# laurabragagnolo/SkelSplat

Hardware: AMD Instinct MI355X
Metric: rendered+backpropagated views/s (differentiable skeletal-Gaussian rasterizer fwd+bwd) (higher is better)
Workload: dtype f32

## Files before the change

### skelsplat_amd/csrc/sks_geom_bwd.inc

```
struct GeomBwdArgs {
    int P, C, W, H;
    unsigned flags;
    const float* vms;
    const float* pms;
    const float* means;
    const float* opac;
    const float* scales;
    const float* rots;
    const float* cov3Dp;
    float smod;
    const int* radii;
    const float* accum;
    int nsplit;
    const double* gt_totals;
    double* loss_sums;
    float* packed;
    float* dmeans3D;
    float* dmeans2D;
    float* dopacity;
    float* dscales;
    float* drots;
    float* dcov3D;
    float* dfeat;
    const uint4* rect = nullptr;
// ... 79 lines not shown
__device__ __forceinline__ void geom_bwd_issue16(const GeomBwdArgs& a, int v, int idx, GeomBwdRaw& r)
{
    const size_t o = (size_t)v * a.P + (idx < a.P ? idx : 0);
    const float* acc = a.accum + o * BWD_SPLITS * (NACC + a.C);
#pragma unroll
    for (int j = 0; j < NACC + 1; j++)
#pragma unroll
        for (int i = 0; i < 4; i++) r.q[j][i] = reinterpret_cast<const float4*>(acc + j * BWD_SPLITS)[i];
}
__device__ __forceinline__ void geom_bwd_sum16(const GeomBwdArgs& a, int idx, const GeomBwdRaw& r, float (&g)[NACC], double& pS,
                                               double& pN)
{
#pragma unroll
    for (int j = 0; j < NACC - 1; j++) {
        float t = 0.0f;
#pragma unroll
        for (int i = 0; i < 4; i++) t += (r.q[j][i].x + r.q[j][i].y) + (r.q[j][i].z + r.q[j][i].w);
        g[j] = t;
    }
    g[NACC - 1] = 0.0f;
    pS = 0.0;
    pN = 0.0;
    if (a.loss_sums && idx < a.P) {
#pragma unroll
        for (int i = 0; i < 4; i++) {
            pS += (double)r.q[7][i].x; pS += (double)r.q[7][i].y; pS += (double)r.q[7][i].z; pS += (double)r.q[7][i].w;
            pN += (double)r.q[8][i].x; pN += (double)r.q[8][i].y; pN += (double)r.q[8][i].z; pN += (double)r.q[8][i].w;
        }
    }
}

struct GeomBwdIn {
    int radius;
    float mean[3], p[7], opac;
};
__device__ __forceinline__ void geom_bwd_fetch(const GeomBwdArgs& a, int v, int idx, GeomBwdIn& in)
{
    const size_t o = (size_t)v * a.P + idx;
    in.radius = a.radii[o];
    in.mean[0] = a.means[3 * idx]; in.mean[1] = a.means[3 * idx + 1]; in.mean[2] = a.means[3 * idx + 2];
    if (a.cov3Dp) {
#pragma unroll
        for (int i = 0; i < 6; i++) in.p[i] = a.cov3Dp[6 * idx + i];
        in.p[6] = 0.0f;
    } else {
        in.p[0] = a.scales[3 * idx]; in.p[1] = a.scales[3 * idx + 1]; in.p[2] = a.scales[3 * idx + 2];
        in.p[3] = a.rots[4 * idx]; in.p[4] = a.rots[4 * idx + 1]; in.p[5] = a.rots[4 * idx + 2]; in.p[6] = a.rots[4 * idx + 3];
    }
    in.opac = a.opac[idx];
}

template <bool PRE = false, class VT = ViewTan>
__device__ __forceinline__ void geom_bwd_finish(const GeomBwdArgs& a, const VT& vt, int v, int idx, const float (&g)[NACC],
                                                double n_view, const GeomBwdIn* pre = nullptr)
{
    const size_t o = (size_t)v * a.P + idx;
    float dmean[3] = { 0, 0, 0 }, dcov[6] = { 0, 0, 0, 0, 0, 0 }, dscale[3] = { 0, 0, 0 }, dq[4] = { 0, 0, 0, 0 };
    float sc[3] = { 0, 0, 0 }, q[4] = { 1, 0, 0, 0 }, qnorm = 1.0f;
    float dop = g[5];
    const float dm2x = g[0], dm2y = g[1];

    if ((PRE ? pre->radius : a.radii[o]) > 0) {
        const float* V = a.vms + 16 * v;
        const float* proj = a.pms + 16 * v;
        const float tan_fovx = vt.x[v], tan_fovy = vt.y[v];
        const float h_y = vt.h[v] / (2.0f * tan_fovy);
        const float h_x = vt.w[v] / (2.0f * tan_fovx);
        const float mean[3] = { PRE ? pre->mean[0] : a.means[3 * idx], PRE ? pre->mean[1] : a.means[3 * idx + 1], PRE ? pre->mean[2] : a.means[3 * idx + 2] };
        float cov3D[6];
        if (a.cov3Dp) {
#pragma unroll
            for (int i = 0; i < 6; i++) cov3D[i] = PRE ? pre->p[i] : a.cov3Dp[6 * idx + i];
        } else {
            const float rs[3] = { PRE ? pre->p[0] : a.scales[3 * idx], PRE ? pre->p[1] : a.scales[3 * idx + 1], PRE ? pre->p[2] : a.scales[3 * idx + 2] };
            const float rq[4] = { PRE ? pre->p[3] : a.rots[4 * idx], PRE ? pre->p[4] : a.rots[4 * idx + 1], PRE ? pre->p[5] : a.rots[4 * idx + 2],
                                  PRE ? pre->p[6] : a.rots[4 * idx + 3] };
            const Activated ac = activate(a.flags & SKS_RAW_PARAMS, 0.0f, rs, rq);
            sc[0] = ac.s[0]; sc[1] = ac.s[1]; sc[2] = ac.s[2];
            q[0] = ac.q[0]; q[1] = ac.q[1]; q[2] = ac.q[2]; q[3] = ac.q[3];
            qnorm = ac.qnorm;
            computeCov3D(sc, a.smod, q, cov3D);
        }
        const float dL_dconic[3] = { g[2], g[3], g[4] };
        Cov2D c;
        cov2d(mean, h_x, h_y, tan_fovx, tan_fovy, cov3D, V, c);
        const float* t = c.t;
        const float x_grad_mul = (c.txtz < -c.limx || c.txtz > c.limx) ? 0 : 1;
        const float y_grad_mul = (c.tytz < -c.limy || c.tytz > c.limy) ? 0 : 1;
        const M3& T = c.T;
        const M3& Wm = c.W;
        const M3& Vrk = c.Vrk;
        float c_xx = c.cov.m[0][0], c_xy = c.cov.m[0][1], c_yy = c.cov.m[1][1];
        constexpr float h_var = 0.3f;
        float d_inside_root = 0.f;
        const bool aa = a.flags & SKS_ANTIALIASING;
        if (aa) {
            const float det_cov = c_xx * c_yy - c_xy * c_xy;
            c_xx += h_var;
            c_yy += h_var;
            const float det_cov_plus_h_cov = c_xx * c_yy - c_xy * c_xy;
            const float h_convolution_scaling = sqrtf(fmaxf(0.000025f, det_cov / det_cov_plus_h_cov));
            const float dL_dopacity_v = dop;
            const float op_raw = PRE ? pre->opac : a.opac[idx];
            const float d_h_convolution_scaling = dL_dopacity_v * ((a.flags & SKS_RAW_PARAMS) ? 1.0f / (1.0f + expf_fixed(-op_raw)) : op_raw);
            dop = dL_dopacity_v * h_convolution_scaling;
            d_inside_root = (det_cov / det_cov_plus_h_cov) <= 0.000025f ? 0.f : d_h_convolution_scaling / (2 * h_convolution_scaling);
        } else {
// ... 38 lines not shown
        const float dL_dJ11 = Wm.m[1][0] * dL_dT10 + Wm.m[1][1] * dL_dT11 + Wm.m[1][2] * dL_dT12;
        const float dL_dJ12 = Wm.m[2][0] * dL_dT10 + Wm.m[2][1] * dL_dT11 + Wm.m[2][2] * dL_dT12;
        const float tz = 1.f / t[2];
        const float tz2 = tz * tz;
        const float tz3 = tz2 * tz;
        const float dL_dtx = x_grad_mul * -h_x * tz2 * dL_dJ02;
        const float dL_dty = y_grad_mul * -h_y * tz2 * dL_dJ12;
        float dL_dtz = -h_x * tz2 * dL_dJ00 - h_y * tz2 * dL_dJ11 + (2 * h_x * t[0]) * tz3 * dL_dJ02 + (2 * h_y * t[1]) * tz3 * dL_dJ12;
        dL_dtz -= g[6] / (t[2] * t[2]);
        dmean[0] = V[0] * dL_dtx + V[1] * dL_dty + V[2] * dL_dtz;
        dmean[1] = V[4] * dL_dtx + V[5] * dL_dty + V[6] * dL_dtz;
        dmean[2] = V[8] * dL_dtx + V[9] * dL_dty + V[10] * dL_dtz;
        float m_hom[4];
        transformPoint4x4(mean, proj, m_hom);
        const float m_w = 1.0f / (m_hom[3] + 0.0000001f);
        const float mul1 = (proj[0] * mean[0] + proj[4] * mean[1] + proj[8] * mean[2] + proj[12]) * m_w * m_w;
        const float mul2 = (proj[1] * mean[0] + proj[5] * mean[1] + proj[9] * mean[2] + proj[13]) * m_w * m_w;
        dmean[0] += (proj[0] * m_w - proj[3] * mul1) * dm2x + (proj[1] * m_w - proj[3] * mul2) * dm2y;
        dmean[1] += (proj[4] * m_w - proj[7] * mul1) * dm2x + (proj[5] * m_w - proj[7] * mul2) * dm2y;
        dmean[2] += (proj[8] * m_w - proj[11] * mul1) * dm2x + (proj[9] * m_w - proj[11] * mul2) * dm2y;
        if (!a.cov3Dp) {
            const float r = q[0], x = q[1], y = q[2], z = q[3];
            const M3 R = quatR(q);
            M3 S = {};
            const float s[3] = { a.smod * sc[0], a.smod * sc[1], a.smod * sc[2] };
            S.m[0][0] = s[0]; S.m[1][1] = s[1]; S.m[2][2] = s[2];
            const M3 M = m3mul(S, R);
            M3 dS;
            dS.m[0][0] = dcov[0]; dS.m[0][1] = 0.5f * dcov[1]; dS.m[0][2] = 0.5f * dcov[2];
            dS.m[1][0] = 0.5f * dcov[1]; dS.m[1][1] = dcov[3]; dS.m[1][2] = 0.5f * dcov[4];
            dS.m[2][0] = 0.5f * dcov[2]; dS.m[2][1] = 0.5f * dcov[4]; dS.m[2][2] = dcov[5];
            M3 M2;
#pragma unroll
            for (int cc = 0; cc < 3; cc++)
#pragma unroll
                for (int rr = 0; rr < 3; rr++) M2.m[cc][rr] = 2.0f * M.m[cc][rr];
            const M3 dL_dM = m3mul(M2, dS);
            const M3 Rt = m3T(R);
            M3 dMt = m3T(dL_dM);
#pragma unroll
            for (int k = 0; k < 3; k++)
                dscale[k] = Rt.m[k][0] * dMt.m[k][0] + Rt.m[k][1] * dMt.m[k][1] + Rt.m[k][2] * dMt.m[k][2];
#pragma unroll
            for (int k = 0; k < 3; k++)
#pragma unroll
                for (int rr = 0; rr < 3; rr++) dMt.m[k][rr] *= s[k];
            dq[0] = 2 * z * (dMt.m[0][1] - dMt.m[1][0]) + 2 * y * (dMt.m[2][0] - dMt.m[0][2]) + 2 * x * (dMt.m[1][2] - dMt.m[2][1]);
            dq[1] = 2 * y * (dMt.m[1][0] + dMt.m[0][1]) + 2 * z * (dMt.m[2][0] + dMt.m[0][2]) + 2 * r * (dMt.m[1][2] - dMt.m[2][1]) - 4 * x * (dMt.m[2][2] + dMt.m[1][1]);
            dq[2] = 2 * x * (dMt.m[1][0] + dMt.m[0][1]) + 2 * r * (dMt.m[2][0] - dMt.m[0][2]) + 2 * z * (dMt.m[1][2] + dMt.m[2][1]) - 4 * y * (dMt.m[2][2] + dMt.m[0][0]);
            dq[3] = 2 * r * (dMt.m[0][1] - dMt.m[1][0]) + 2 * x * (dMt.m[2][0] + dMt.m[0][2]) + 2 * y * (dMt.m[1][2] + dMt.m[2][1]) - 4 * z * (dMt.m[1][1] + dMt.m[0][0]);
        }
    }
    if (a.dmeans3D) { a.dmeans3D[3 * o] = dmean[0]; a.dmeans3D[3 * o + 1] = dmean[1]; a.dmeans3D[3 * o + 2] = dmean[2]; }
    if (a.dmeans2D) { a.dmeans2D[3 * o] = dm2x; a.dmeans2D[3 * o + 1] = dm2y; a.dmeans2D[3 * o + 2] = 0.0f; }
    const bool rawg = (a.flags & SKS_RAW_PARAMS) && (a.flags & SKS_RAW_GRADS);
    if (a.dopacity) {
        float oj = 1.0f;
        if (rawg) {
            const float so = 1.0f / (1.0f + expf_fixed(-(PRE ? pre->opac : a.opac[idx])));
            oj = so * (1.0f - so);
        }
        a.dopacity[o] = dop * oj;
    }
    if (a.dcov3D) {
#pragma unroll
        for (int i = 0; i < 6; i++) a.dcov3D[6 * o + i] = dcov[i];
    }
    if (a.dscales) {
#pragma unroll
        for (int k = 0; k < 3; k++) a.dscales[3 * o + k] = dscale[k] * (rawg ? sc[k] : 1.0f);
    }
    if (a.drots) {
        float dot = 0.0f;
#pragma unroll
        for (int k = 0; k < 4; k++) dot += q[k] * dq[k];
#pragma unroll
        for (int k = 0; k < 4; k++) a.drots[4 * o + k] = rawg ? (dq[k] - q[k] * dot) / qnorm : dq[k];
    }
    if (a.packed) {
        float scl = 1.0f;
        if (a.loss_sums) scl = (float)(1.0 / (n_view < 1.0 ? 1.0 : n_view));
        float* pk = a.packed + o * 11;
        const bool raw = a.flags & SKS_RAW_PARAMS;
        pk[0] = dmean[0] * scl; pk[1] = dmean[1] * scl; pk[2] = dmean[2] * scl;
#pragma unroll
        for (int k = 0; k < 3; k++) pk[3 + k] = dscale[k] * (raw ? sc[k] : 1.0f) * scl;
        float dot = 0.0f;
#pragma unroll
        for (int k = 0; k < 4; k++) dot += q[k] * dq[k];
#pragma unroll
        for (int k = 0; k < 4; k++) pk[6 + k] = (raw ? (dq[k] - q[k] * dot) / qnorm : dq[k]) * scl;
        float oj = 1.0f;
        if (raw) {
            const float so = 1.0f / (1.0f + expf_fixed(-(PRE ? pre->opac : a.opac[idx])));
            oj = so * (1.0f - so);
        }
        pk[10] = dop * oj * scl;
    }
}

__global__ __launch_bounds__(256) void k_geom_bwd(GeomBwdArgs a, ViewTan vt)
{
    const int idx = blockIdx.x * 256 + threadIdx.x;
    const int v = blockIdx.y;
    float g[NACC];
    double pS, pN;
// ... 25 lines not shown
    const int idx = blockIdx.x * GEOMB_G + tid;
    GeomBwdIn in;
    const bool mine = tid < GEOMB_G && idx < a.P;
    if (mine) geom_bwd_fetch(a, v, idx, in);
    {
        const int gi = tid >> 2, st = tid & 3;
        const int gidx = blockIdx.x * GEOMB_G + gi;
        float sum[NACC];
#pragma unroll
        for (int k = 0; k < NACC; k++) sum[k] = 0.0f;
        if (gidx < a.P) {
            const size_t o = (size_t)v * a.P + gidx;
            const uint4 r = a.rect[o];
            const int n = BIN_ROWS * (int)((r.z - r.x) * (r.w - r.y));
            const size_t s0 = BIN_ROWS * (size_t)a.goff[o], send = BIN_ROWS * a.cap;
            const float4* rows = reinterpret_cast<const float4*>(a.part + (size_t)v * a.cap * BIN_ROWS * NACC);
            for (int i = st; i < n; i += 16) {
                float4 q[4][2];
#pragma unroll
                for (int u = 0; u < 4; u++) {
                    const bool on = i + 4 * u < n && s0 + i + 4 * u < send;
                    q[u][0] = on ? rows[(s0 + i + 4 * u) * 2] : make_float4(0, 0, 0, 0);
                    q[u][1] = on ? rows[(s0 + i + 4 * u) * 2 + 1] : make_float4(0, 0, 0, 0);
                }
#pragma unroll
                for (int u = 0; u < 4; u++) {
                    sum[0] += q[u][0].x; sum[1] += q[u][0].y; sum[2] += q[u][0].z; sum[3] += q[u][0].w;
                    sum[4] += q[u][1].x; sum[5] += q[u][1].y; sum[6] += q[u][1].z;
                }
            }
        }
        float4* sg = reinterpret_cast<float4*>(s_g[gi][st]);
        sg[0] = make_float4(sum[0], sum[1], sum[2], sum[3]);
        sg[1] = make_float4(sum[4], sum[5], sum[6], 0.0f);
    }
    __syncthreads();
    if (!mine) return;
    float g[NACC];
#pragma unroll
    for (int k = 0; k < NACC - 1; k++) g[k] = (s_g[tid][0][k] + s_g[tid][1][k]) + (s_g[tid][2][k] + s_g[tid][3][k]);
    g[NACC - 1] = 0.0f;
    if (a.bin_hdr[0]) {
#pragma unroll
        for (int k = 0; k < NACC - 1; k++) g[k] = __int_as_float(0x7fc00000);
    }
    if (a.dfeat) {
        const size_t o = (size_t)v * a.P + idx;
        const float* acc = a.accum + o * (NACC + a.C);
        for (int ch = 0; ch < a.C; ch++) a.dfeat[o * a.C + ch] = acc[NACC + ch];
    }
    geom_bwd_finish<true>(a, vt, v, idx, g, 1.0, &in);
}

template <class... PF>
__global__ __launch_bounds__(256) void k_geom_bwd_all(GeomBwdArgs a, ViewTan vt, int V, float* __restrict__ mean_out, PF... pf)
{
    static_assert(sizeof...(PF) <= 1, "at most one PreFill");
    if constexpr (sizeof...(PF) == 1) {
        if (blockIdx.x > 0) {
            prefill_block((pf, ...), blockIdx.x - 1u);
            return;
        }
    }
    const int t = threadIdx.x;
    const int v = t / a.P, idx = t - v * a.P;
    const bool live = v < V;
    float g[NACC];
    double pS, pN;
    if (a.dfeat) geom_bwd_dfeat(a, 0, V * a.P, t, 256);
    if (live) {
        geom_bwd_load<false>(a, v, idx, g, pS, pN);
        geom_bwd_finish(a, vt, v, idx, g, 1.0);
    }
    __syncthreads();
    if (t < a.P) {
        float m[3] = { 0.0f, 0.0f, 0.0f };
        for (int w0 = 0; w0 < V; w0 += 4) {
            float tv[4][3];
#pragma unroll
            for (int j = 0; j < 4; j++) {
                const float* gm = a.dmeans3D + ((size_t)(w0 + j < V ? w0 + j : V - 1) * a.P + t) * 3;
                tv[j][0] = gm[0]; tv[j][1] = gm[1]; tv[j][2] = gm[2];
            }
#pragma unroll
            for (int j = 0; j < 4; j++)
                if (w0 + j < V) { m[0] += tv[j][0]; m[1] += tv[j][1]; m[2] += tv[j][2]; }
        }
        mean_out[3 * t] = m[0] / (float)V; mean_out[3 * t + 1] = m[1] / (float)V; mean_out[3 * t + 2] = m[2] / (float)V;
    }
}
__global__ void k_mean_views(int V, int P, const float* __restrict__ dmeans3D, float* __restrict__ mean_out, int world = 1)
{
    const int i = blockIdx.x * blockDim.x + threadIdx.x;
    if (i >= 3 * P) return;
    const int vmax = (V + world - 1) / world;
    float m = 0.0f;
    for (int w0 = 0; w0 < V; w0 += 8) {
        float t[8];
#pragma unroll
        for (int j = 0; j < 8; j++) {
            const int w = w0 + j < V ? w0 + j : V - 1;
            const int row = world == 1 ? w : (w % world) * vmax + w / world;
            t[j] = dmeans3D[(size_t)row * P * 3 + i];
        }
#pragma unroll
        for (int j = 0; j < 8; j++)
            if (w0 + j < V) m += t[j];
    }
    mean_out[i] = m / (float)V;
}

template <bool ES = false, class VT = ViewTan>
__global__ __launch_bounds__(256) void k_step_tail(GeomBwdArgs ga, VT vt, sksloop::AdamArgs aa, int V, Geom g, int* radii)
{
    __shared__ float s_xyz[256 * 3];
    __shared__ float s_hyp[6];
    __shared__ double s_d[4];
    __shared__ int s_it[2];
    __shared__ float s_np[64 * 11];
    const int tid = threadIdx.x, lane = tid & 63, wv = tid >> 6;
    const int P = ga.P;
    const int f = blockIdx.x, vb = f * V;
    if (f) {
        ga.means += (size_t)f * P * 3; ga.opac += (size_t)f * P; ga.scales += (size_t)f * P * 3; ga.rots += (size_t)f * P * 4;
        aa.grads += (size_t)vb * P * 11; aa.slots += (size_t)vb * P * 3;
        aa.xyz += (size_t)f * P * 3; aa.scaling += (size_t)f * P * 3; aa.rotation += (size_t)f * P * 4; aa.opacity += (size_t)f * P;
        aa.m += (size_t)f * P * 11; aa.vv += (size_t)f * P * 11; aa.counters += 2 * f;
    }
    if constexpr (std::is_same<VT, ViewTanDev>::value) {
        const double* r = vt.sched + 5 * (size_t)f;
        aa.log_lr_init = r[0]; aa.log_lr_final = r[1]; aa.lr_delay_mult = r[2];
        aa.lr_delay_steps = (int)r[3]; aa.lr_max_steps = (int)r[4];
        aa.lr_init = r[0] == -INFINITY ? 0.0 : 1.0;
        aa.lr_final = r[1] == -INFINITY ? 0.0 : 1.0;
    }
    if constexpr (ES) {
        aa.es_state += (size_t)f * (2 + 2 * aa.es_window);
        if (aa.es_host_flag) aa.es_host_flag += f;
        if (aa.es_state[1] != 0) return;
// ... 47 lines not shown
```

### skelsplat_amd/csrc/sks_geom_fwd.inc

```
template <class VT>
__device__ __forceinline__ uint4 geom_fwd_one(int P, const VT& vt, const float* __restrict__ vms,
                                              const float* __restrict__ pms, const float* __restrict__ means,
                                              const float* __restrict__ opac, const float* __restrict__ scales,
                                              const float* __restrict__ rots, const float* __restrict__ cov3Dp,
                                              float smod, unsigned flags, const Geom& g, int* __restrict__ radii,
                                              int v, int idx, bool live, bool store = true)
{
    const size_t o = (size_t)v * P + (live ? idx : 0);
    const float* V = vms + 16 * v;
    const float* PM = pms + 16 * v;
    const float tan_fovx = vt.x[v], tan_fovy = vt.y[v];
    const int W = vt.w[v], H = vt.h[v];
    const float focal_y = H / (2.0f * tan_fovy);
    const float focal_x = W / (2.0f * tan_fovx);
    const int gx = (W + TILE - 1) / TILE, gy = (H + TILE - 1) / TILE;

    int radius_out = 0;
    uint4 rect = make_uint4(0, 0, 0, 0);
    float4 co = make_float4(0, 0, 0, 0), xyd = make_float4(0, 0, 1.0f, 1.0f);

    const int li = live ? idx : 0;
    const float p_orig[3] = { means[3 * li], means[3 * li + 1], means[3 * li + 2] };
    float p_view[3];
    transformPoint4x3(p_orig, V, p_view);
// ... 24 lines not shown
        if (flags & SKS_ANTIALIASING) h_convolution_scaling = sqrtf(fmaxf(0.000025f, det_cov / det_cov_plus_h_cov));
        const float det = det_cov_plus_h_cov;
        if (det != 0.0f) {
            const float det_inv = 1.f / det;
            const float conic[3] = { cov_z * det_inv, -cov_y * det_inv, cov_x * det_inv };
            const float mid = 0.5f * (cov_x + cov_z);
            const float lambda1 = mid + sqrtf(fmaxf(0.1f, mid * mid - det));
            const float lambda2 = mid - sqrtf(fmaxf(0.1f, mid * mid - det));
            const float my_radius = ceilf(3.f * sqrtf(fmaxf(lambda1, lambda2)));
            const float px = ndc2Pix(p_proj[0], W), py = ndc2Pix(p_proj[1], H);
            int xmin, ymin, xmax, ymax;
            getRect(px, py, (int)my_radius, gx, gy, xmin, ymin, xmax, ymax);
            if ((xmax - xmin) * (ymax - ymin) != 0) {
                radius_out = (int)my_radius;
                rect = make_uint4(xmin, ymin, xmax, ymax);
                const float op_raw = opac[li];
                const float op = (flags & SKS_RAW_PARAMS) ? 1.0f / (1.0f + expf_fixed(-op_raw)) : op_raw;
                co = make_float4(conic[0], conic[1], conic[2], op * h_convolution_scaling);
                xyd = make_float4(px, py, p_view[2], 1 / p_view[2]);
            }
        }
    }
    if (live && store) {
        radii[o] = radius_out;
        g.co[o] = co;
        g.xyd[o] = xyd;
        g.rect[o] = rect;
    }
    return rect;
}

#ifndef SKS_GEOM_COVER_THREADS
#define SKS_GEOM_COVER_THREADS 256
#endif
__device__ __forceinline__ void geom_fwd_block(uint32_t* s_cov, int bx, int v, int pz, int P, int W, int H, const ViewTan& vt, const float* __restrict__ vms,
                                               const float* __restrict__ pms, const float* __restrict__ means,
                                               const float* __restrict__ opac, const float* __restrict__ scales,
                                               const float* __restrict__ rots, const float* __restrict__ cov3Dp,
                                               float smod, unsigned flags, const Geom& g, int* __restrict__ radii, int vf,
                                               uint32_t* __restrict__ count, uint32_t* __restrict__ touched,
                                               const float* __restrict__ features, int C,
                                               uint2* __restrict__ fmask, uint32_t* __restrict__ bin_hdr, int cover_planes)
{
    const int idx = bx * blockDim.x + threadIdx.x;
    const bool live = idx < P;
    if (vf > 0) {
        const int fr = v / vf;
        means += (size_t)fr * P * 3;
        opac += (size_t)fr * P;
        if (scales) scales += (size_t)fr * P * 3;
        if (rots) rots += (size_t)fr * P * 4;
        if (cov3Dp) cov3Dp += (size_t)fr * P * 6;
    }
    const uint4 rect = geom_fwd_one(P, vt, vms, pms, means, opac, scales, rots, cov3Dp, smod, flags, g, radii, v, idx, live, pz == 0);
    if (bin_hdr && bx == 0 && v == 0 && pz == 0 && threadIdx.x < 64) bin_hdr[threadIdx.x] = 0u;
    if (count) {
        const int wt = (int)(rect.z - rect.x), n = wt * (int)(rect.w - rect.y);
        if (live) touched[(size_t)v * P + idx] = (uint32_t)n;
        if (live && v == 0) {
            unsigned fm = 0u;
            float f0 = 0.0f;
            for (int ch = C - 1; ch >= 0; ch--) {
                const float f = features[(size_t)idx * C + ch];
                if (f != 0.0f) { fm |= 1u << ch; f0 = f; }
            }
            fmask[idx] = make_uint2(fm, __float_as_uint(f0));
        }
    }
    if (g.cover) {
        const int gy = (H + TILE - 1) / TILE;
        const int cw = cover_cw(W), pw = gy * cw;
        for (int i = threadIdx.x; i < pw; i += blockDim.x) s_cov[i] = 0u;
        __syncthreads();
        bool mine = live && rect.z > rect.x && rect.w > rect.y;
        if (mine && cover_planes && pz < C) mine = features[(size_t)idx * C + pz] != 0.0f;
        if (mine) {
#pragma nounroll
            for (unsigned y = rect.y; y < rect.w; y++) {
                atomicOr(&s_cov[y * cw], 1u);
#pragma nounroll
                for (unsigned w0 = rect.x >> 5; w0 <= (rect.z - 1u) >> 5; w0++) {
                    const unsigned lo = max(rect.x, w0 << 5) & 31u, hi = min(rect.z - 1u, (w0 << 5) + 31u) & 31u;
                    atomicOr(&s_cov[y * cw + 1 + w0], (0xffffffffu >> (31u - hi)) & (0xffffffffu << lo));
                }
            }
        }
        __syncthreads();
        uint32_t* out = g.cover + ((size_t)v * (cover_planes ? C + 1 : 1) + (cover_planes ? pz : 0)) * pw;
        for (int i = threadIdx.x; i < pw; i += blockDim.x) out[i] = s_cov[i];
    }
}

__global__ __launch_bounds__(SKS_GEOM_COVER_THREADS > 256 ? SKS_GEOM_COVER_THREADS : 256) void k_geom_fwd(int P, int W, int H, ViewTan vt, const float* __restrict__ vms,
                                                   const float* __restrict__ pms, const float* __restrict__ means,
                                                   const float* __restrict__ opac, const float* __restrict__ scales,
                                                   const float* __restrict__ rots, const float* __restrict__ cov3Dp,
                                                   float smod, unsigned flags, Geom g, int* __restrict__ radii, int vf,
                                                   uint32_t* __restrict__ count = nullptr, uint32_t* __restrict__ touched = nullptr,
                                                   const float* __restrict__ features = nullptr, int C = 0,
                                                   uint2* __restrict__ fmask = nullptr, uint32_t* __restrict__ bin_hdr = nullptr,
                                                   int cover_planes = 0)
{
    __shared__ uint32_t s_cov[COVER_MAX_WORDS];
    geom_fwd_block(s_cov, blockIdx.x, blockIdx.y, blockIdx.z, P, W, H, vt, vms, pms, means, opac, scales, rots, cov3Dp, smod, flags, g, radii, vf,
                   count, touched, features, C, fmask, bin_hdr, cover_planes);
}

__global__ __launch_bounds__(256) void k_geom_fwd_dv(int P, ViewTanDev vt, const float* __restrict__ vms, const float* __restrict__ pms,
                                                      const float* __restrict__ means, const float* __restrict__ opac,
                                                      const float* __restrict__ scales, const float* __restrict__ rots,
                                                      const float* __restrict__ cov3Dp, float smod, unsigned flags, Geom g,
                                                      int* __restrict__ radii, int vf)
{
    const int idx = blockIdx.x * 256 + threadIdx.x;
    const int v = blockIdx.y;
    if (vf > 0) {
        const int fr = v / vf;
        means += (size_t)fr * P * 3;
        opac += (size_t)fr * P;
        if (scales) scales += (size_t)fr * P * 3;
        if (rots) rots += (size_t)fr * P * 4;
        if (cov3Dp) cov3Dp += (size_t)fr * P * 6;
    }
    geom_fwd_one(P, vt, vms, pms, means, opac, scales, rots, cov3Dp, smod, flags, g, radii, v, idx, idx < P);
}

__global__ void k_mark_visible(int P, const float* __restrict__ means, const float* __restrict__ V,
                               uint8_t* __restrict__ present)
// ... 9 lines not shown
```

### skelsplat_amd/csrc/sks_raster.hip

```cpp
#include <hip/hip_runtime.h>
#include <hip/hip_ext.h>
#include <stdarg.h>
#include <stdlib.h>
#include <stdio.h>
#include <string.h>
#include <type_traits>

#include "../../include/skelsplat_hip.h"
#include "sks_math.h"
#include "sks_loop_dev.h"

using namespace sks;

namespace {

#include "sks_common.inc"
#include "sks_geom_fwd.inc"
#include "sks_fwd_small.inc"
#include "sks_bwd_small.inc"
#include "sks_geom_bwd.inc"
#include "sks_binned.inc"

inline int pick_cg(int C) { return C <= 4 ? 4 : C <= 16 ? 16 : C <= 20 ? 20 : 32; }

// ... 128 lines not shown

inline int bwd_tile_blocks()
{
    static const int n = [] {
        int dev = 0, cus = 256;
        if (hipGetDevice(&dev) == hipSuccess) {
            hipDeviceProp_t pr;
            if (hipGetDeviceProperties(&pr, dev) == hipSuccess && pr.multiProcessorCount > 0) cus = pr.multiProcessorCount;
        }
        const char* e = getenv("SKS_BWD_TILE_BLOCKS");
        return (e && atoi(e) > 0) ? atoi(e) : cus * BWD_TILE_BLOCKS_PER_CU;
    }();
    return n;
}

inline int bwd_wave_groups(int V, int P, unsigned flags)
{
    unsigned t = (flags >> SKS_BWD_WG_SHIFT) & 7u;
    static const int env = [] { const char* e = getenv("SKS_BWD_WG"); return e ? atoi(e) : 0; }();
    if (!t && env > 0) t = (unsigned)env;
    if (t) return t > 5 ? 1 : (BWD_SPLITS >> (t - 1));
    const int pairs = V * P;
    return pairs <= BWD_WG_PAIRS16 ? 16 : (pairs <= BWD_WG_PAIRS8 ? 8 : 4);
}

template <bool ES = false>
inline void launch_bwd_loss(const BwdArgs& a, const ViewTan& vt, const ViewOff& vo, dim3 grid, int cg, hipStream_t st)
{
    if (a.hm_row) {
        switch (cg) {
            case 4: hipLaunchKernelGGL((k_render_bwd_wave<4, false, true, true, ES>), grid, dim3(256), 0, st, a, vt, vo); break;
            case 16: hipLaunchKernelGGL((k_render_bwd_wave<16, false, true, true, ES>), grid, dim3(256), 0, st, a, vt, vo); break;
            case 20: hipLaunchKernelGGL((k_render_bwd_wave<20, false, true, true, ES>), grid, dim3(256), 0, st, a, vt, vo); break;
            default: hipLaunchKernelGGL((k_render_bwd_wave<32, false, true, true, ES>), grid, dim3(256), 0, st, a, vt, vo); break;
        }
        return;
    }
    switch (cg) {
        case 4: hipLaunchKernelGGL((k_render_bwd_wave<4, false, true, false, ES>), grid, dim3(256), 0, st, a, vt, vo); break;
        case 16: hipLaunchKernelGGL((k_render_bwd_wave<16, false, true, false, ES>), grid, dim3(256), 0, st, a, vt, vo); break;
        case 20: hipLaunchKernelGGL((k_render_bwd_wave<20, false, true, false, ES>), grid, dim3(256), 0, st, a, vt, vo); break;
        default: hipLaunchKernelGGL((k_render_bwd_wave<32, false, true, false, ES>), grid, dim3(256), 0, st, a, vt, vo); break;
    }
}

struct PrefillReq {
    float* color;
    float* invdepth;
    int planes_wave, planes_geom;
};
#ifndef SKS_PREFILL_PASSES
#define SKS_PREFILL_PASSES 2
#endif
inline int prefill_passes()
{
    static const int n = [] { const char* e = getenv("SKS_PREFILL_PB"); return (e && atoi(e) > 0) ? atoi(e) : SKS_PREFILL_PASSES; }();
    return n > 32 ? 32 : n;
}
inline bool prefill_possible(int P, int W, int H, unsigned flags)
{
    return P >= 1 && P <= 64 && P <= SKS_SMALL_P && !(flags & (SKS_FORCE_BINNED | SKS_NO_NT_STORES | SKS_DEBUG_SYNC | (1u << 20))) &&
           (W % 4 == 0 || (W % 4 == 2 && H % 2 == 0));
}
bool prefill_cut(PreFill& f, float* color, float* invdepth, int V, int C, int W, int H, int zid0, int nz, long long per_unit, long long max_units)
{
    const int gy = (H + TILE - 1) / TILE;
    const bool lines = color && invdepth && (((uintptr_t)color | (uintptr_t)invdepth) & 127u) == 0;
    const int lead = (lines && (long long)H * W % 32 == 0 && TILE * W % 32 == 0) ? 0 : 31;
    const int passes = (TILE * W + lead + 1023) / 1024;
    const int pb = prefill_passes();
    const int fsplit = (passes + pb - 1) / pb;
    const long long rows = (long long)fsplit * gy, nfill = rows * nz;
    if (zid0 < 0 || nz < 1 || zid0 + nz > (C + 1) * V || nfill * rows >= (1ll << 32) || (nfill + per_unit - 1) / per_unit > max_units) return false;
    f = PreFill{ color, invdepth, C, W, H, gy, zid0, (unsigned)nfill, fsplit, pb, 0, ((1u << 20) + (unsigned)C) / (unsigned)(C + 1),
                 rows > 1 ? magic32((unsigned)rows) : 0u, fsplit > 1 ? magic32((unsigned)fsplit) : 0u };
    return true;
}

inline bool bwd_small_wave(int P, unsigned flags) { return P <= 64 && !(flags & (1u << 20)); }

template <int CG>
void launch_bwd_small(const BwdArgs& a, const ViewTan& vt, const ViewOff& vo, int V, int gy, bool dfeat, hipStream_t st,
                      const ProfScope& prof, const PreFill* pf = nullptr)
{
    (void)gy;
    if (bwd_small_wave(a.P, a.flags)) {
        dim3 grid(a.P, V, bwd_wave_groups(V, a.P, a.flags));
        if (pf) {
            PreFill f = *pf;
            f.zs = (int)grid.z;
            grid.z += (unsigned)((f.nfill + (unsigned)(a.P * V) - 1) / (unsigned)(a.P * V));
            if (dfeat) SKS_LAUNCH(prof, (k_render_bwd_wave<CG, true, false, false, false, PreFill>), grid, dim3(256), 0, st, a, vt, vo, f);
            else SKS_LAUNCH(prof, (k_render_bwd_wave<CG, false, false, false, false, PreFill>), grid, dim3(256), 0, st, a, vt, vo, f);
            return;
        }
        if (dfeat) SKS_LAUNCH(prof, (k_render_bwd_wave<CG, true, false>), grid, dim3(256), 0, st, a, vt, vo);
        else SKS_LAUNCH(prof, (k_render_bwd_wave<CG, false, false>), grid, dim3(256), 0, st, a, vt, vo);
        return;
    }
    dim3 grid(a.P, V, BWD_SPLITS);
    const size_t lds = GatherLds<CG>::bytes((a.P + 15) & ~15, CG, a.C);
    if (lds > 48 * 1024) {
        (void)hipFuncSetAttribute(reinterpret_cast<const void*>(&k_render_bwd_gather<CG, true>),
                                  hipFuncAttributeMaxDynamicSharedMemorySize, (int)lds);
        (void)hipFuncSetAttribute(reinterpret_cast<const void*>(&k_render_bwd_gather<CG, false>),
                                  hipFuncAttributeMaxDynamicSharedMemorySize, (int)lds);
    }
    if (dfeat) SKS_LAUNCH(prof, (k_render_bwd_gather<CG, true>), grid, dim3(256), lds, st, a);
    else SKS_LAUNCH(prof, (k_render_bwd_gather<CG, false>), grid, dim3(256), lds, st, a);
}

__global__ void k_spin_us(unsigned long long ticks)
{
    const unsigned long long t0 = wall_clock64();
    while (wall_clock64() - t0 < ticks) __builtin_amdgcn_s_sleep(8);
}

struct FwdHook {
    hipEvent_t geom_done;
    int (*after_geom)(void* ctx);
    int (*after_group)(void* ctx, int g, int v0, int nv);
    void* ctx;
};
// ... 237 lines not shown

extern "C" {

int sks_forward(int V, int P, int C, int W, int H, const float* viewmatrix, const float* projmatrix,
                const float* tanfovx, const float* tanfovy, const float* means3D, const float* features,
                const float* opacities, const float* scales, const float* rotations, const float* cov3D_precomp,
                float scale_modifier, unsigned flags, float* out_color, float* out_invdepth, int* radii, void* geom,
                void* binning, size_t bin_capacity, int* num_rendered_dev, float* final_T, uint32_t* n_contrib,
                void* stream)
{
    return forward_impl(V, P, C, W, H, viewmatrix, projmatrix, tanfovx, tanfovy, means3D, features, opacities, scales, rotations,
                        cov3D_precomp, scale_modifier, flags, out_color, out_invdepth, radii, geom, binning, bin_capacity,
                        num_rendered_dev, final_T, n_contrib, stream, nullptr);
}

}

namespace {

constexpr unsigned BWD_RENDER = 1u, BWD_GEOM = 2u;
int backward_impl(int V, int P, int C, int W, int H, const float* viewmatrix, const float* projmatrix,
                  const float* tanfovx, const float* tanfovy, const float* bg, const float* means3D,
                  const float* features, const float* opacities, const float* scales, const float* rotations,
                  const float* cov3D_precomp, float scale_modifier, unsigned flags, const int* radii, const void* geom,
                  const void* binning, size_t bin_capacity, const float* dL_dout_color, const float* dL_dout_invdepth,
                  void* accum, float* dL_dmeans3D, float* dL_dmeans2D, float* dL_dopacity, float* dL_dscales,
                  float* dL_drotations, float* dL_dcov3D, float* dL_dfeatures, float* dL_dmeans3D_mean, void* stream,
                  unsigned phases, int group, const PrefillReq* pre = nullptr)
{
    if (int rc = check_common(V, P, C, W, H)) return rc;
    if (P == 0) return 0;
    hipStream_t st = (hipStream_t)stream;
    if (!viewmatrix || !projmatrix || !tanfovx || !tanfovy || !means3D || !features || !opacities || !radii ||
        !geom || !dL_dout_color || !accum || !dL_dmeans3D || !dL_dmeans2D || !dL_dopacity)
        return fail(-2, "missing required pointer");
    if (!cov3D_precomp && (!scales || !rotations)) return fail(-2, "need scales+rotations or cov3D_precomp");
    ViewTan vt;
    ViewOff vo;
    fill_views(vt, &vo, V, C, W, H, tanfovx, tanfovy, nullptr, nullptr);
    Geom g = geom_from(const_cast<void*>(geom), V, P, W, H);
    const int gx = (W + TILE - 1) / TILE, gy = (H + TILE - 1) / TILE, NT = gx * gy;
    BwdArgs a{ P, C, W, H, flags, g, features, bg, dL_dout_color, dL_dout_invdepth, (float*)accum, nullptr, nullptr };
    const int cg = pick_cg(C);
    const bool dfeat = dL_dfeatures != nullptr;
    const bool small = P <= SKS_SMALL_P && !(flags & SKS_FORCE_BINNED);
    int vg = V, ng = 1;
    if (!small) bin_groups(flags, V, vg, ng);
    if (group >= ng) return fail(-1, "view group %d of %d", group, ng);
    const bool geom_all = dL_dmeans3D_mean && V * P <= 256 && small;
    PreFill pfw{}, pfg{};
    bool have_pfw = false, have_pfg = false;
    if (pre && pre->planes_wave + pre->planes_geom > 0) {
        const int planes = (C + 1) * V, n = pre->planes_wave + pre->planes_geom;
        const int n_geom = geom_all ? pre->planes_geom : 0, nw = n - n_geom;
        if (nw > 0) {
            if (!prefill_cut(pfw, pre->color, pre->invdepth, V, C, W, H, planes - n, nw, (long long)P * V, 65535 - BWD_SPLITS))
                return fail(-1, "sks_backward_prefill: %d planes of %dx%d do not fit the compositing backward's launch", nw, W, H);
            have_pfw = true;
        }
        if (n_geom > 0) {
            if (!prefill_cut(pfg, pre->color, pre->invdepth, V, C, W, H, planes - n_geom, n_geom, 1, (1ll << 31) - 2))
                return fail(-1, "sks_backward_prefill: %d planes of %dx%d do not fit the geometry backward's launch", n_geom, W, H);
            have_pfg = true;
        }
        if (prof_next_forward_sampled()) prof_park_begin(st);
    }
    if ((phases & BWD_RENDER) && small) {
        ProfScope prof(1, st, true);
        const PreFill* pf = have_pfw ? &pfw : nullptr;
        switch (cg) {
            case 4: launch_bwd_small<4>(a, vt, vo, V, gy, dfeat, st, prof, pf); break;
            case 16: launch_bwd_small<16>(a, vt, vo, V, gy, dfeat, st, prof, pf); break;
            case 20: launch_bwd_small<20>(a, vt, vo, V, gy, dfeat, st, prof, pf); break;
            default: launch_bwd_small<32>(a, vt, vo, V, gy, dfeat, st, prof, pf); break;
        }
        STAGE_CHECK("render-backward(small)");
    } else if (phases & BWD_RENDER) {
        if (!binning) return fail(-2, "binned path needs the forward's binning buffer");
        Bin b = bin_from(const_cast<void*>(binning), V, P, NT, bin_capacity);
        BinView bv = bin_view(b, NT, bin_capacity);
        if (dfeat && group <= 0) HIP_TRY(hipMemsetAsync(accum, 0, (size_t)V * P * (NACC + C) * sizeof(float), st));
        dim3 grid(bwd_tile_blocks());
        const unsigned magic_nt = (unsigned)(((1ull << 32) + (unsigned)NT - 1) / (unsigned)NT), magic_gx = (unsigned)(((1ull << 32) + (unsigned)gx - 1) / (unsigned)gx);
        const bool extra = bg != nullptr || dL_dout_invdepth != nullptr;
        for (int gi = group < 0 ? 0 : group; gi < (group < 0 ? ng : group + 1); gi++) {
            const uint4* tl = b.tlist + (size_t)gi * vg * NT;
            const uint32_t* hd = b.hdr + gi * BIN_CLASSES;
            ProfScope prof(1, st);
            if (dfeat) hipLaunchKernelGGL((k_render_bwd_tile<true, true>), grid, dim3(BWD_TILE_THREADS), 0, st, a, bv, gx, V, magic_nt, magic_gx, tl, hd);
            else if (extra) hipLaunchKernelGGL((k_render_bwd_tile<false, true>), grid, dim3(BWD_TILE_THREADS), 0, st, a, bv, gx, V, magic_nt, magic_gx, tl, hd);
            else hipLaunchKernelGGL((k_render_bwd_tile<false, false>), grid, dim3(BWD_TILE_THREADS), 0, st, a, bv, gx, V, magic_nt, magic_gx, tl, hd);
        }
        STAGE_CHECK("render-backward(binned)");
    }
    if (!(phases & BWD_GEOM)) return 0;
    GeomBwdArgs ga{ P, C, W, H, flags, viewmatrix, projmatrix, means3D, opacities, scales, rotations, cov3D_precomp,
                    scale_modifier, radii, (const float*)accum, small ? BWD_SPLITS : 0, nullptr, nullptr, nullptr, dL_dmeans3D, dL_dmeans2D, dL_dopacity, dL_dscales,
                    dL_drotations, dL_dcov3D, dL_dfeatures };
    if (!small) {
        Bin b = bin_from(const_cast<void*>(binning), V, P, NT, bin_capacity);
        ga.rect = g.rect;
        ga.goff = b.goff;
        ga.part = b.part;
        ga.cap = bin_capacity;
        ga.bin_hdr = b.hdr;
    }
    if (geom_all) {
        if (have_pfg) hipLaunchKernelGGL((k_geom_bwd_all<PreFill>), dim3(1u + pfg.nfill), dim3(256), 0, st, ga, vt, V, dL_dmeans3D_mean, pfg);
        else hipLaunchKernelGGL((k_geom_bwd_all<>), dim3(1), dim3(256), 0, st, ga, vt, V, dL_dmeans3D_mean);
    } else {
        if (small) hipLaunchKernelGGL(k_geom_bwd, dim3((P + 255) / 256, V), dim3(256), 0, st, ga, vt);
        else {
            const int v0 = group < 0 ? 0 : group * vg, nv = group < 0 ? V : ((V - v0 < vg) ? V - v0 : vg);
            ga.v0 = v0;
// ... 540 lines not shown
```

Baseline: 70050.

## Split geometry-backward split-sum across three threads per pair and keep dmean in LDS

The single-block all-views geometry backward now assigns three threads to each (view, point) pair when 3*V*P fits in a block. Each thread reduces part of the per-split accumulator using float4 loads, and the partial sums are combined in shared memory. Per-view mean gradients are also kept in LDS for the cross-view mean, so they are no longer re-read from global memory. A separate geom prefill pass count knob is added, and the forward hoists the feature load for the coverage test. This shortens the serial load-and-reduce latency of the tiny backward kernel, at the cost of extra LDS and the restriction to small V*P. Prefill planes are routed to the geom kernel only when the three-thread path applies.

Measured after the change: 69880. Within noise of the previous version (-0.2%).

```diff
diff --git a/skelsplat_amd/csrc/sks_geom_bwd.inc b/skelsplat_amd/csrc/sks_geom_bwd.inc
--- a/skelsplat_amd/csrc/sks_geom_bwd.inc
+++ b/skelsplat_amd/csrc/sks_geom_bwd.inc
@@ -155,7 +155,7 @@
 
 template <bool PRE = false, class VT = ViewTan>
 __device__ __forceinline__ void geom_bwd_finish(const GeomBwdArgs& a, const VT& vt, int v, int idx, const float (&g)[NACC],
-                                                double n_view, const GeomBwdIn* pre = nullptr)
+                                                double n_view, const GeomBwdIn* pre = nullptr, float* dmean_out = nullptr)
 {
     const size_t o = (size_t)v * a.P + idx;
     float dmean[3] = { 0, 0, 0 }, dcov[6] = { 0, 0, 0, 0, 0, 0 }, dscale[3] = { 0, 0, 0 }, dq[4] = { 0, 0, 0, 0 };
@@ -300,6 +300,7 @@
         }
     }
     if (a.dmeans3D) { a.dmeans3D[3 * o] = dmean[0]; a.dmeans3D[3 * o + 1] = dmean[1]; a.dmeans3D[3 * o + 2] = dmean[2]; }
+    if (dmean_out) { dmean_out[0] = dmean[0]; dmean_out[1] = dmean[1]; dmean_out[2] = dmean[2]; }
     if (a.dmeans2D) { a.dmeans2D[3 * o] = dm2x; a.dmeans2D[3 * o + 1] = dm2y; a.dmeans2D[3 * o + 2] = 0.0f; }
     const bool rawg = (a.flags & SKS_RAW_PARAMS) && (a.flags & SKS_RAW_GRADS);
     if (a.dopacity) {
@@ -431,6 +432,8 @@
     geom_bwd_finish<true>(a, vt, v, idx, g, 1.0, &in);
 }
 
+constexpr int GEOM_ALL3_PAIRS = 85;
+__host__ __device__ inline bool geom_all_three(int V, int P) { return 3 * V * P <= 256; }
 template <class... PF>
 __global__ __launch_bounds__(256) void k_geom_bwd_all(GeomBwdArgs a, ViewTan vt, int V, float* __restrict__ mean_out, PF... pf)
 {
@@ -441,29 +444,73 @@
             return;
         }
     }
-    const int t = threadIdx.x;
-    const int v = t / a.P, idx = t - v * a.P;
-    const bool live = v < V;
-    float g[NACC];
-    double pS, pN;
-    if (a.dfeat) geom_bwd_dfeat(a, 0, V * a.P, t, 256);
-    if (live) {
-        geom_bwd_load<false>(a, v, idx, g, pS, pN);
-        geom_bwd_finish(a, vt, v, idx, g, 1.0);
+    __shared__ float s_g[GEOM_ALL3_PAIRS][NACC];
+    __shared__ GeomBwdIn s_in[GEOM_ALL3_PAIRS];
+    __shared__ float s_dm[256 * 3];
+    const int t = threadIdx.x, n = V * a.P;
+    a.packed = nullptr;
+    a.loss_sums = nullptr;
+    if (a.dfeat) geom_bwd_dfeat(a, 0, n, t, 256);
+    if (geom_all_three(V, a.P)) {
+        const int pair = t / 3, k = t - 3 * pair;
+        const float* acc = a.accum + (size_t)(pair < n ? pair : 0) * BWD_SPLITS * (NACC + a.C);
+        const int j0 = k == 0 ? 0 : (k == 1 ? 2 : 5);
+        static_assert(BWD_SPLITS == 16 && NACC == 8, "4 x float4 per value, 7 values");
+        float4 q[3][4];
+#pragma unroll
+        for (int u = 0; u < 2; u++)
+#pragma unroll
+            for (int i = 0; i < 4; i++) q[u][i] = reinterpret_cast<const float4*>(acc + (j0 + u) * BWD_SPLITS)[i];
+        if (k == 1) {
+#pragma unroll
+            for (int i = 0; i < 4; i++) q[2][i] = reinterpret_cast<const float4*>(acc + 4 * BWD_SPLITS)[i];
+        } else {
+#pragma unroll
+            for (int i = 0; i < 4; i++) q[2][i] = make_float4(0, 0, 0, 0);
+        }
+        const bool lead = t < n;
+        const int v = t / a.P, idx = t - v * a.P;
+        if (lead) {
+            GeomBwdIn in;
+            geom_bwd_fetch(a, v, idx, in);
+            s_in[t] = in;
+        }
+        float s[3];
+#pragma unroll
+        for (int u = 0; u < 3; u++) {
+            float x = 0.0f;
+#pragma unroll
+            for (int i = 0; i < 4; i++) x += (q[u][i].x + q[u][i].y) + (q[u][i].z + q[u][i].w);
+            s[u] = x;
+        }
+        if (pair < n) {
+            s_g[pair][j0] = s[0];
+            s_g[pair][j0 + 1] = s[1];
+            if (k == 1) s_g[pair][4] = s[2];
+        }
+        __syncthreads();
+        if (lead) {
+            float g[NACC];
+#pragma unroll
+            for (int j = 0; j < NACC - 1; j++) g[j] = s_g[t][j];
+            g[NACC - 1] = 0.0f;
+            geom_bwd_finish<true>(a, vt, v, idx, g, 1.0, &s_in[t], s_dm + 3 * t);
+        }
+    } else if constexpr (sizeof...(PF) == 0) {
+        const int v = t / a.P, idx = t - v * a.P;
+        if (v < V) {
+            float g[NACC];
+            double pS, pN;
+            geom_bwd_load<false>(a, v, idx, g, pS, pN);
+            geom_bwd_finish(a, vt, v, idx, g, 1.0, nullptr, s_dm + 3 * t);
+        }
     }
     __syncthreads();
     if (t < a.P) {
         float m[3] = { 0.0f, 0.0f, 0.0f };
-        for (int w0 = 0; w0 < V; w0 += 4) {
-            float tv[4][3];
-#pragma unroll
-            for (int j = 0; j < 4; j++) {
-                const float* gm = a.dmeans3D + ((size_t)(w0 + j < V ? w0 + j : V - 1) * a.P + t) * 3;
-                tv[j][0] = gm[0]; tv[j][1] = gm[1]; tv[j][2] = gm[2];
-            }
-#pragma unroll
-            for (int j = 0; j < 4; j++)
-                if (w0 + j < V) { m[0] += tv[j][0]; m[1] += tv[j][1]; m[2] += tv[j][2]; }
+        for (int w = 0; w < V; w++) {
+            const float* gm = s_dm + (w * a.P + t) * 3;
+            m[0] += gm[0]; m[1] += gm[1]; m[2] += gm[2];
         }
         mean_out[3 * t] = m[0] / (float)V; mean_out[3 * t + 1] = m[1] / (float)V; mean_out[3 * t + 2] = m[2] / (float)V;
     }
diff --git a/skelsplat_amd/csrc/sks_geom_fwd.inc b/skelsplat_amd/csrc/sks_geom_fwd.inc
--- a/skelsplat_amd/csrc/sks_geom_fwd.inc
+++ b/skelsplat_amd/csrc/sks_geom_fwd.inc
@@ -100,6 +100,8 @@
         if (rots) rots += (size_t)fr * P * 4;
         if (cov3Dp) cov3Dp += (size_t)fr * P * 6;
     }
+    float feat_pz = 1.0f;
+    if (g.cover && live && cover_planes && pz < C) feat_pz = features[(size_t)idx * C + pz];
     const uint4 rect = geom_fwd_one(P, vt, vms, pms, means, opac, scales, rots, cov3Dp, smod, flags, g, radii, v, idx, live, pz == 0);
     if (bin_hdr && bx == 0 && v == 0 && pz == 0 && threadIdx.x < 64) bin_hdr[threadIdx.x] = 0u;
     if (count) {
@@ -121,7 +123,7 @@
         for (int i = threadIdx.x; i < pw; i += blockDim.x) s_cov[i] = 0u;
         __syncthreads();
         bool mine = live && rect.z > rect.x && rect.w > rect.y;
-        if (mine && cover_planes && pz < C) mine = features[(size_t)idx * C + pz] != 0.0f;
+        if (mine && cover_planes && pz < C) mine = feat_pz != 0.0f;
         if (mine) {
 #pragma nounroll
             for (unsigned y = rect.y; y < rect.w; y++) {
diff --git a/skelsplat_amd/csrc/sks_raster.hip b/skelsplat_amd/csrc/sks_raster.hip
--- a/skelsplat_amd/csrc/sks_raster.hip
+++ b/skelsplat_amd/csrc/sks_raster.hip
@@ -204,9 +204,14 @@
 #ifndef SKS_PREFILL_PASSES
 #define SKS_PREFILL_PASSES 2
 #endif
-inline int prefill_passes()
-{
-    static const int n = [] { const char* e = getenv("SKS_PREFILL_PB"); return (e && atoi(e) > 0) ? atoi(e) : SKS_PREFILL_PASSES; }();
+#ifndef SKS_PREFILL_PASSES_GEOM
+#define SKS_PREFILL_PASSES_GEOM SKS_PREFILL_PASSES
+#endif
+inline int prefill_passes(bool geom = false)
+{
+    static const int env[2] = { [] { const char* e = getenv("SKS_PREFILL_PB"); return e ? atoi(e) : 0; }(),
+                                [] { const char* e = getenv("SKS_PREFILL_PB_GEOM"); return e ? atoi(e) : 0; }() };
+    const int n = (geom && env[1] > 0) ? env[1] : env[0] > 0 ? env[0] : geom ? SKS_PREFILL_PASSES_GEOM : SKS_PREFILL_PASSES;
     return n > 32 ? 32 : n;
 }
 inline bool prefill_possible(int P, int W, int H, unsigned flags)
@@ -214,13 +219,13 @@
     return P >= 1 && P <= 64 && P <= SKS_SMALL_P && !(flags & (SKS_FORCE_BINNED | SKS_NO_NT_STORES | SKS_DEBUG_SYNC | (1u << 20))) &&
            (W % 4 == 0 || (W % 4 == 2 && H % 2 == 0));
 }
-bool prefill_cut(PreFill& f, float* color, float* invdepth, int V, int C, int W, int H, int zid0, int nz, long long per_unit, long long max_units)
+bool prefill_cut(PreFill& f, float* color, float* invdepth, int V, int C, int W, int H, int zid0, int nz, long long per_unit, long long max_units, bool geom = false)
 {
     const int gy = (H + TILE - 1) / TILE;
     const bool lines = color && invdepth && (((uintptr_t)color | (uintptr_t)invdepth) & 127u) == 0;
     const int lead = (lines && (long long)H * W % 32 == 0 && TILE * W % 32 == 0) ? 0 : 31;
     const int passes = (TILE * W + lead + 1023) / 1024;
-    const int pb = prefill_passes();
+    const int pb = prefill_passes(geom);
     const int fsplit = (passes + pb - 1) / pb;
     const long long rows = (long long)fsplit * gy, nfill = rows * nz;
     if (zid0 < 0 || nz < 1 || zid0 + nz > (C + 1) * V || nfill * rows >= (1ll << 32) || (nfill + per_unit - 1) / per_unit > max_units) return false;
@@ -564,14 +569,14 @@
     bool have_pfw = false, have_pfg = false;
     if (pre && pre->planes_wave + pre->planes_geom > 0) {
         const int planes = (C + 1) * V, n = pre->planes_wave + pre->planes_geom;
-        const int n_geom = geom_all ? pre->planes_geom : 0, nw = n - n_geom;
+        const int n_geom = (geom_all && geom_all_three(V, P)) ? pre->planes_geom : 0, nw = n - n_geom;
         if (nw > 0) {
             if (!prefill_cut(pfw, pre->color, pre->invdepth, V, C, W, H, planes - n, nw, (long long)P * V, 65535 - BWD_SPLITS))
                 return fail(-1, "sks_backward_prefill: %d planes of %dx%d do not fit the compositing backward's launch", nw, W, H);
             have_pfw = true;
         }
         if (n_geom > 0) {
-            if (!prefill_cut(pfg, pre->color, pre->invdepth, V, C, W, H, planes - n_geom, n_geom, 1, (1ll << 31) - 2))
+            if (!prefill_cut(pfg, pre->color, pre->invdepth, V, C, W, H, planes - n_geom, n_geom, 1, (1ll << 31) - 2, true))
                 return fail(-1, "sks_backward_prefill: %d planes of %dx%d do not fit the geometry backward's launch", n_geom, W, H);
             have_pfg = true;
         }
```
